# eldar/deepcut-cnn

Hardware: AMD Instinct MI355X
Metric: images/sec, DeeperCut ResNet-152 FCN forward (prob+loc_pred+next_pred), whole node (higher is better)
Workload: dtype f32

## Files before the change

deepcut-cnn_amd/csrc/c_api.cpp:

```cpp
#include <hip/hip_runtime_api.h>

#include <algorithm>
#include <cstdio>
#include <cstring>
#include <memory>
#include <string>
#include <vector>

#include "../../include/deepcut_hip.h"
#include "net.h"

using namespace dc;


namespace {
thread_local std::string g_err;
int fail(int code, const std::string& msg) {
  g_err = msg;
  return code;
}
template <typename F>
int guard(F&& f) {
  try {
    f();
// ... 581 lines not shown
const char* dc_conv_variant_name(int i) { return i >= 0 && i < dc::conv_num_variants() ? dc::conv_variant(i).name : nullptr; }
int dc_conv_variant_esize(int i) { return i >= 0 && i < dc::conv_num_variants() ? dc::conv_variant_esize(i) : 0; }
int dc_conv_bf16_variant_count(void) { return dc::conv_num_bf16_variants(); }
const char* dc_conv_bf16_variant_name(int i) {
  return i >= 0 && i < dc::conv_num_bf16_variants() ? dc::conv_variant(dc::kBf16Variant0 + i).name : nullptr;
}
int dc_wino_half_pack(const float* g, int cout, int cin, int rowscale, float* out, float* row_scale) {
  REQUIRE(g);
  REQUIRE(out);
  REQUIRE(row_scale);
  if (cout <= 0 || cin <= 0 || cout % 32 || cin % 16) return fail(DC_EINVAL, "dc_wino_half_pack: cout must be a multiple of 32, cin of 16");
  return guard([&] { dc::wino_half_pack_filters(g, cout, cin, rowscale != 0, out, row_scale); });
}

int dc_wino_blocks(const char* tile, int tiles_y, int tiles_x) {
  if (!tile || tiles_y < 1 || tiles_x < 1) return -1;
  try {
    return (int)dc::wino_form_blocks(dc::variant_by_name(tile), tiles_y, tiles_x);
  } catch (...) {
    return -1;
  }
}

int dc_stream1x1_pack(const float* g, int cout, int k, float* out) {
  if (!g || !out) return fail(DC_EINVAL, "dc_stream1x1_pack: null pointer");
  if (cout <= 0 || k <= 0 || cout % 32 || k % 16) return fail(DC_EINVAL, "dc_stream1x1_pack: cout must be a multiple of 32, k of 16");
  return guard([&] { dc::stream1x1_pack_filters(g, cout, k, out); });
}

int dc_stream1x1f_pack(const float* g, int cout, int k, float* out) {
  if (!g || !out) return fail(DC_EINVAL, "dc_stream1x1f_pack: null pointer");
  if (cout <= 0 || k <= 0 || cout % 16 || k % 16) return fail(DC_EINVAL, "dc_stream1x1f_pack: cout and k must be multiples of 16");
  return guard([&] { dc::stream1x1f_pack_filters(g, cout, k, out); });
}

int dc_stem7x7_pack(const float* g, int c, float* out) {
  if (!g || !out) return fail(DC_EINVAL, "dc_stem7x7_pack: null pointer");
  if (c < 1 || c > 4) return fail(DC_EINVAL, "dc_stem7x7_pack: 1 to 4 input channels");
  return guard([&] { dc::stem7x7_pack_filters(g, c, out); });
}

namespace {
inline NetGroup* G(dc_group* g) { return reinterpret_cast<NetGroup*>(g); }
}
int dc_group_create(dc_net* const* nets, int n, dc_group** out) {
  REQUIRE(nets);
// ... 206 lines not shown
```

deepcut-cnn_amd/csrc/forms.cpp:

```cpp
#include <cstring>
#include <string>

#include "kernels.h"

namespace dc {

static const char* const kWinoSlots[7] = {"index setup", "first loads issued", "two stages in LDS", "K loop", "partials to LDS + barrier",
                                          "inverse transform + epilogue constants", "shortcut + stores"};
static const char* const kStreamSlots[7] = {"prologue requests issued", "first stage + filters landed", "the first D steps", "the other steps",
                                            "drain", "-", "exit"};
static constexpr ConvForm kForms[kNumForms] = {
    {kWinoVariant, "wino_f23", "wino_f23<4x8x16>", kElemF32, kForm3x3, 8, kWinoSlots, wino_eligible, wino_grid, launch_wino_f23,
     false, false, nullptr, nullptr, kWinoVariant16, "DC_WINOGRAD"},
    {kWinoVariant16, "wino_f23_w16", "wino_f23<4x8x16_w16>", kElemF32, kForm3x3, 16, kWinoSlots, wino_eligible, wino_grid, launch_wino_f23_w16,
     false, false, nullptr, nullptr, kWinoVariant, "DC_WINOGRAD"},
    {kWinoHalf, "wino_h23", "wino_h23<2x4x8x64>", kElemF16, kForm3x3, 8, kWinoSlots, wino_half_eligible, wino_half_grid, launch_wino_half,
     true, true, nullptr, nullptr, -1, "DC_WINOGRAD"},
    {kStreamHalf, "ws1x1", "ws1x1<32xN>", kElemF16, kForm1x1, 4, kStreamSlots, stream1x1_eligible, stream1x1_grid, launch_stream1x1,
     false, true, stream1x1_prepare_multi, launch_stream1x1_multi, -1, "DC_STREAM1X1"},
    {kStemHalf, "stem7x7", "stem7x7<8x64>", kElemF16, kFormStem, 4, kWinoSlots, stem7x7_eligible, stem7x7_grid, launch_stem7x7,
     false, false, nullptr, nullptr, -1, "DC_STEM"},
    {kStreamFloat, "ws1x1f", "ws1x1f<16xN>", kElemF32, kForm1x1, 4, kStreamSlots, stream1x1f_eligible, stream1x1f_grid, launch_stream1x1f,
     false, true, nullptr, nullptr, -1, "DC_STREAM1X1"},
    {kStemFloat, "ws7x7f", "ws7x7f<16x64>", kElemF32, kFormStem, 4, kStreamSlots, stem_ws_eligible, stem_ws_grid, launch_stem_ws,
     false, true, nullptr, nullptr, -1, "DC_STEM"},
    {kWinoVariant56, "wino_f23_5x6", "wino_f23<5x6x16>", kElemF32, kForm3x3, 8, kWinoSlots, wino_eligible, wino_grid_5x6, launch_wino_f23_5x6,
     false, false, nullptr, nullptr, kWinoVariant56x16, "DC_WINOGRAD", wino_fewer_blocks},
    {kWinoVariant56x16, "wino_f23_5x6_w16", "wino_f23<5x6x16_w16>", kElemF32, kForm3x3, 16, kWinoSlots, wino_eligible, wino_grid_5x6, launch_wino_f23_5x6_w16,
     false, false, nullptr, nullptr, kWinoVariant56, "DC_WINOGRAD", wino_fewer_blocks},
    {kStreamBf16, "bs1x1", "bs1x1<32xN>", kElemBF16, kForm1x1, 4, kStreamSlots, stream1x1_bf16_eligible, stream1x1_grid, launch_stream1x1_bf16,
     false, true, stream1x1_bf16_prepare_multi, launch_stream1x1_bf16_multi, -1, "DC_STREAM1X1_BF16", nullptr, 0},
    {kStemBf16, "bs7x7", "bs7x7<8x64>", kElemBF16, kFormStem, 4, kWinoSlots, stem7x7_bf16_eligible, stem7x7_grid, launch_stem7x7_bf16,
     false, false, nullptr, nullptr, -1, "DC_STEM_BF16", nullptr, 0},
};

static constexpr bool forms_in_variant_order() {
  for (int i = 0; i < kNumForms; ++i)
    if (kForms[i].variant != kFormVariant0 + i) return false;
  return true;
}
static_assert(forms_in_variant_order(), "row i of kForms is variant kFormVariant0 + i");

const ConvForm* conv_form(int variant) {
  return variant >= kFormVariant0 && variant < kFormVariant0 + kNumForms ? &kForms[variant - kFormVariant0] : nullptr;
}

const char* variant_name(int v) {
  const ConvForm* f = conv_form(v);
  return f ? f->name : conv_variant(v).name;
}
int variant_by_name(const char* name) {
  for (const ConvForm& f : kForms)
    if (std::strcmp(name, f.name) == 0) return f.variant;
  return conv_variant_by_name(name);
}
std::string variant_kernel_label(int v) {
// ... 14 lines not shown
```

deepcut-cnn_amd/csrc/kernels.h:

```cpp
#pragma once
#include <cstddef>
#include <cstdint>
#include <string>

namespace dc {

constexpr int kMaxTaps = 32;

void dc_magic(unsigned d, unsigned (&mg)[2]);
bool xcd_map_on();

enum ElemKind { kElemF32 = 0, kElemF16 = 1, kElemBF16 = 2 };
inline int elem_kind_size(int kind) { return kind == kElemF32 ? 4 : 2; }
inline const char* elem_kind_name(int kind) { return kind == kElemF16 ? "f16" : kind == kElemBF16 ? "bf16" : "f32"; }

constexpr int kMaxClasses = 4;
struct ConvClass {
  int nty, ntx, dy0, ddy, x0, ddx, Ktot, x_bias;
  int OH, OW, M;
  int tiles_m;
  unsigned div_ohw[2];
  unsigned div_ow[2];
  long w_off;
  long y_off;
// ... 46 lines not shown
  int y_pix_stride;
  const void* resid;
  const float* scale;
  const float* shift;
  int relu;
  int sigmoid_ch;
  int xcd_on;
  int xcd_lgx;
  int tiles_m;
  unsigned div_rw[2][2];
  unsigned div_ohw[2];
  unsigned div_ow[2];
  unsigned div_tn[2];
  int tiles_n;
  long long* dbg;
  int w_TY, w_TX, w_NBY, w_NBX, w_nblk;
  unsigned w_div_nblk[2], w_div_nbyx[2], w_div_dd[2], w_div_d[2], w_div_nbx[2];
  int wide_epi;
  int vec_epi;
  int dense_x;
  int dense_y;
  int ncls;
  int mc_lgx;
  ConvClass cls[kMaxClasses];
  int nprob;
  int ekind;
};
struct ConvMultiArgs {
  ConvGemmParams p;
  ConvMultiTable t;
};
static_assert(sizeof(ConvMultiArgs) <= 4096, "HIP kernel arguments are limited to 4 KB");

struct ConvVariant {
  const char* name;
  int BM, BN, WR, WC, WK;
};
int conv_num_variants();
const ConvVariant& conv_variant(int i);
int conv_variant_bk(int i);
int conv_variant_esize(int i);
constexpr int kBf16Variant0 = 2000;
int conv_num_bf16_variants();
inline bool is_bf16_variant(int v) { return v >= kBf16Variant0 && v < kBf16Variant0 + conv_num_bf16_variants(); }
int conv_variant_ekind(int v);
bool conv_variant_exists(int v);
const int* conv_variants_of(int ekind, int* count);
int conv_variant_by_name(const char* name);
bool conv_variant_multiclass(int i);
long conv_grid(const ConvGemmParams& p, int variant);
int launch_conv_gemm(const ConvGemmParams& p, int variant, void* stream);
long prepare_conv_multi(ConvGemmParams& p, ConvMultiTable& table, int nprob, int variant);
bool conv_variant_multiproblem(int i);
int launch_conv_multi(const ConvMultiArgs& a, int variant, long grid, void* stream);

bool wino_eligible(const ConvGemmParams& p);
bool wino_same3x3(const ConvGemmParams& p);
ConvGemmParams wino_launch_params(const ConvGemmParams& p, long grid, int bty, int btx, int blocks_per_wg);
long wino_grid(const ConvGemmParams& p);
long wino_grid_5x6(const ConvGemmParams& p);
bool wino_fewer_blocks(const ConvGemmParams& p);
int launch_wino_f23(const ConvGemmParams& p, void* stream);
int launch_wino_f23_w16(const ConvGemmParams& p, void* stream);
int launch_wino_f23_5x6(const ConvGemmParams& p, void* stream);
int launch_wino_f23_5x6_w16(const ConvGemmParams& p, void* stream);
long wino_blocks(int TY, int TX, int bty, int btx);
long wino_form_blocks(int variant, int TY, int TX);
size_t wino_packed_floats(int Cout, int Cin);
void wino_pack_filters(const float* g, int Cout, int Cin, float* out);
bool wino_half_eligible(const ConvGemmParams& p);
long wino_half_grid(const ConvGemmParams& p);
size_t wino_half_packed_elems(int Cout, int Cin);
void wino_half_pack_filters(const float* g, int Cout, int Cin, bool rowscale, float* out, float* row_scale);
int launch_wino_half(const ConvGemmParams& p, void* stream);
bool stream1x1_eligible(const ConvGemmParams& p);
long stream1x1_grid(const ConvGemmParams& p);
size_t stream1x1_packed_elems(int Cout, int K);
void stream1x1_pack_filters(const float* g, int Cout, int K, float* out);
int launch_stream1x1(const ConvGemmParams& p, void* stream);
bool stream1x1f_eligible(const ConvGemmParams& p);
long stream1x1f_grid(const ConvGemmParams& p);
size_t stream1x1f_packed_elems(int Cout, int K);
void stream1x1f_pack_filters(const float* g, int Cout, int K, float* out);
int launch_stream1x1f(const ConvGemmParams& p, void* stream);
// ... 7 lines not shown
size_t stem7x7_packed_elems();
void stem7x7_pack_filters(const float* g, int C, float* out);
int launch_stem7x7(const ConvGemmParams& p, void* stream);
long stream1x1_prepare_multi(const ConvGemmParams& p, const ConvMultiTable& tb, int nprob);
int launch_stream1x1_multi(const ConvMultiArgs& a, void* stream);
bool stream1x1_bf16_eligible(const ConvGemmParams& p);
int launch_stream1x1_bf16(const ConvGemmParams& p, void* stream);
long stream1x1_bf16_prepare_multi(const ConvGemmParams& p, const ConvMultiTable& tb, int nprob);
int launch_stream1x1_bf16_multi(const ConvMultiArgs& a, void* stream);
bool stem7x7_bf16_eligible(const ConvGemmParams& p);
int launch_stem7x7_bf16(const ConvGemmParams& p, void* stream);

constexpr int kWinoVariant = 1000;
constexpr int kWinoVariant16 = 1001;
constexpr int kWinoHalf = 1002;
constexpr int kStreamHalf = 1003;
constexpr int kStemHalf = 1004;
constexpr int kStreamFloat = 1005;
constexpr int kStemFloat = 1006;
constexpr int kWinoVariant56 = 1007;
constexpr int kWinoVariant56x16 = 1008;
constexpr int kStreamBf16 = 1009;
constexpr int kStemBf16 = 1010;
constexpr int kFormVariant0 = kWinoVariant, kNumForms = 11;
enum FormGeometry { kForm3x3, kForm1x1, kFormStem };
struct ConvForm {
  int variant;
  const char *name, *label;
  int ekind, geometry, waves;
  const char* const* timing_slots;
  bool (*eligible)(const ConvGemmParams& p);
  long (*grid)(const ConvGemmParams& p);
  int (*launch)(const ConvGemmParams& p, void* stream);
  bool own_scale;
  bool merges;
  long (*prepare_multi)(const ConvGemmParams& p, const ConvMultiTable& tb, int nprob);
  int (*launch_multi)(const ConvMultiArgs& a, void* stream);
  int sibling;
  const char* env;
  bool (*offered)(const ConvGemmParams& p) = nullptr;
  int env_default = -1;
};
const ConvForm* conv_form(int variant);

const char* variant_name(int v);
int variant_by_name(const char* name);
std::string variant_kernel_label(int v);
// ... 97 lines not shown
```

deepcut-cnn_amd/csrc/wino_f32.hip:

```cpp
#include <hip/hip_runtime.h>

#include "conv_gemm.h"
#include "kernel_prims.h"
#include "kernels.h"

namespace dc {

namespace {
constexpr int WBTY = 4, WBTX = 8, WBN = 16, WKC = 32;
constexpr int WPSTR = WKC + 4;
constexpr int WPITCH = 672;
constexpr int WNTH = 512;
template <int FR_, int FC_, bool SIDE_, int PITCH_>
struct WinoGeom {
  static constexpr int FR = FR_, FC = FC_, NT = FR_ * FC_, PITCH = PITCH_;
  static constexpr bool SIDE = SIDE_;
  static constexpr int BTY = SIDE_ ? FR_ : 2 * FR_, BTX = SIDE_ ? 2 * FC_ : FC_;
  static constexpr int RH = 2 * BTY + 2, RW = 2 * BTX + 2;
  static constexpr int STAGE = RH * PITCH_ + 8;
  static constexpr int frow(int tf) { return SIDE_ ? 0 : FR_ * tf; }
  static constexpr int fcol(int tf) { return SIDE_ ? FC_ * tf : 0; }
  static constexpr int trow(int tf, int q) { return frow(tf) + q / FC_; }
  static constexpr int tcol(int tf, int q) { return fcol(tf) + q % FC_; }
  static constexpr bool conflict_free() {
    for (int tf = 0; tf < 2; ++tf)
      for (int flip = 0; flip < 2; ++flip) {
        bool seen[16] = {};
        for (int q = 0; q < NT; ++q) {
          const int slot = ((2 * trow(tf, q) * PITCH_ + 2 * tcol(tf, q) * WPSTR) / 4 + ((q >= 4 && q < 12) != (flip != 0) ? 1 : 0)) & 15;
          if (seen[slot]) return false;
          seen[slot] = true;
        }
      }
    return true;
  }
  static_assert(NT <= 16 && PITCH_ >= RW * WPSTR && WPSTR == 36 && conflict_free(), "conflict-free ds_read_b128 layout (see above)");
  static_assert(PITCH_ % 4 == 0 && WPSTR % 4 == 0 && STAGE % 4 == 0, "16-byte units");
};
using WinoG48 = WinoGeom<WBTY / 2, WBTX, false, WPITCH>;
using WinoG56 = WinoGeom<5, 3, true, 524>;
static_assert(WinoG48::BTY == 4 && WinoG48::BTX == 8 && WinoG48::RH == 10 && WinoG48::RW == 18, "the 4 x 8 block");
static_assert(WinoG56::BTY == 5 && WinoG56::BTX == 6 && WinoG56::RH == 12 && WinoG56::RW == 14, "the 5 x 6 block");
__device__ __forceinline__ f32x2 wlo(f32x4 v) { return __builtin_shufflevector(v, v, 0, 1); }
__device__ __forceinline__ f32x2 whi(f32x4 v) { return __builtin_shufflevector(v, v, 2, 3); }
}

template <int NG, class G>
__global__ __launch_bounds__(WNTH * NG, 4) void wino_f23_kernel(const ConvGemmParams p) {
  constexpr int NTH = WNTH * NG;
  constexpr int BTY = G::BTY, BTX = G::BTX, WRH = G::RH, WRW = G::RW, PITCH = G::PITCH, WSTAGE = G::STAGE;
  constexpr int WNLD = (WRH * WRW * (WKC / 4) + NTH - 1) / NTH;
  const long long t_entry = (long long)__builtin_amdgcn_s_memrealtime();
  DC_KARG_TOUCH(ka0, ka1, ka2, ka3, ka4);
  __shared__ __attribute__((aligned(16))) float stage[3][WSTAGE];
  float (*part)[4][2][2][4][64] = reinterpret_cast<float (*)[4][2][2][4][64]>(&stage[0][0]);
  static_assert(sizeof(float) * NG * 4 * 2 * 2 * 4 * 64 <= sizeof(stage), "partials must fit in the staging ring");
  static_assert(2 * sizeof(stage) <= 160 * 1024, "two workgroups per CU");
  const int t = threadIdx.x, lane = t & 63, wave = t >> 6;
  auto stamp = [&](int slot) {
    if (p.dbg && lane == 0) {
      long long* d = p.dbg + ((long)blockIdx.x * (8 * NG) + wave) * 12;
      d[slot] = (long long)__builtin_readcyclecounter();
      if (slot == 0) d[8] = t_entry, d[10] = (long long)__builtin_amdgcn_s_memrealtime();
      if (slot == 7) d[9] = (long long)__builtin_amdgcn_s_memrealtime();
    }
  };
  stamp(0);
  const int C = p.klen, H = p.x_rows, W = p.x_rowlen / p.klen;
  const int d = p.ddy;
  const int NBY = p.w_NBY, NBX = p.w_NBX;
  const int nblk = p.w_nblk;
  int lb = blockIdx.x;
  if (p.xcd_on) {
    const int g8 = gridDim.x >> 3, r8 = gridDim.x & 7, q = blockIdx.x & 7;
    lb = q * g8 + min(q, r8) + (blockIdx.x >> 3);
  }
  const int nt = dc_fastdiv(lb, p.w_div_nblk), blk = lb - nt * nblk;
  const int nph = dc_fastdiv(blk, p.w_div_nbyx), brem = blk - nph * (NBY * NBX);
  const int n = dc_fastdiv(nph, p.w_div_dd), ph = nph - n * (d * d);
  const int phy = dc_fastdiv(ph, p.w_div_d), phx = ph - phy * d;
  const int by = dc_fastdiv(brem, p.w_div_nbx), bx = brem - by * NBX;
  const int oy0 = 2 * BTY * by - 1, ox0 = 2 * BTX * bx - 1;
  DC_KARG_HOLD(ka0, ka1, ka2, ka3, ka4);
  const int kg = lane >> 4;
  const int grp = NG == 1 ? 0 : __builtin_amdgcn_readfirstlane(wave >> 3);
  const int i = wave & 3, tf = (wave >> 2) & 1;
  const int ra = i == 0 ? 0 : (i == 2 ? 2 : 1), rb = i == 0 ? 2 : (i == 1 ? 2 : (i == 2 ? 1 : 3));
  const float sb = i == 1 ? 1.f : -1.f;
  const __amdgpu_buffer_rsrc_t xr = dc_rsrc(reinterpret_cast<const float*>(p.x) + (long)n * p.x_img_stride, 0x7fffffffu);
  const __amdgpu_buffer_rsrc_t ur = dc_rsrc(p.w, 0x7fffffffu);
  unsigned gofs[WNLD];
  int sofs[WNLD];
#pragma unroll
  for (int q = 0; q < WNLD; ++q) {
    const int e = t + q * NTH;
    const int pix = e / (WKC / 4), cq = e % (WKC / 4);
    const int py = pix / WRW, px = pix % WRW;
    const int iy = phy + d * (oy0 + py), ix = phx + d * (ox0 + px);
    const bool ok = pix < WRH * WRW && oy0 + py >= 0 && ox0 + px >= 0 && iy < H && ix < W;
    gofs[q] = ok ? (unsigned)(iy * p.x_row_stride + ix * C + cq * 4) * 4u : kOOB;
    sofs[q] = (pix < WRH * WRW ? py * PITCH + px * WPSTR + cq * 4 : WSTAGE - 8 + (t & 1) * 4) >> 2;
  }
  const int qt = G::NT < 16 ? min(lane & 15, G::NT - 1) : lane & 15;
  const int r = qt / G::FC, c = G::fcol(tf) + qt % G::FC;
  const int ofs_a = (2 * (G::frow(tf) + r) + ra) * PITCH + 2 * c * WPSTR + kg * 4;
  const int ofs_b = (2 * (G::frow(tf) + r) + rb) * PITCH + 2 * c * WPSTR + kg * 4;
  f32x4 acc[4];
#pragma unroll
  for (int j = 0; j < 4; ++j) acc[j] = f32x4{0.f, 0.f, 0.f, 0.f};
  const unsigned uvo = ((unsigned)((nt * 4 + i) * (C / 16)) * (4 * 64 * 4) + (unsigned)lane * 4u) * 4u;
  f32x4 g[WNLD], b[2][4], da[4], db[4];
  auto gload = [&](int K) {
#pragma unroll
    for (int q = 0; q < WNLD; ++q) g[q] = dc_bload4(xr, gofs[q], (unsigned)(K * WKC * 4));
  };
  auto sstore = [&](int buf) {
#pragma unroll
    for (int q = 0; q < WNLD; ++q) reinterpret_cast<f32x4*>(&stage[buf][0])[sofs[q]] = g[q];
  };
  auto bload = [&](int slot, int k16) {
#pragma unroll
    for (int j = 0; j < 4; ++j) b[slot][j] = dc_bload4(ur, uvo + (unsigned)j * 1024u, (unsigned)k16 * 4096u);
  };
  auto lread = [&](int buf, int h) {
#pragma unroll
    for (int c4 = 0; c4 < 4; ++c4) {
      da[c4] = *reinterpret_cast<const f32x4*>(&stage[buf][ofs_a + c4 * WPSTR + h * 16]);
      db[c4] = *reinterpret_cast<const f32x4*>(&stage[buf][ofs_b + c4 * WPSTR + h * 16]);
    }
// ... 79 lines not shown
  stamp(4);
  __syncthreads();
#pragma unroll
  for (int r4 = 0; r4 < 4; ++r4) {
    part[grp][i][0][tf][r4][lane] = acc[0][r4] + acc[1][r4] + acc[2][r4];
    part[grp][i][1][tf][r4][lane] = acc[1][r4] - acc[2][r4] - acc[3][r4];
  }
  __syncthreads();
  stamp(5);
  const int a = (wave >> 1) & 1, bq = wave & 1;
  float* yb = reinterpret_cast<float*>(p.y);
  const float* rbp = reinterpret_cast<const float*>(p.resid);
  stamp(6);
#pragma unroll
  for (int rr = 0; rr < 4 / NG; ++rr) {
    const int r4 = NG == 1 ? rr : 2 * grp + rr;
    float p0 = part[0][0][bq][tf][r4][lane], p1 = part[0][1][bq][tf][r4][lane], p2 = part[0][2][bq][tf][r4][lane], p3 = part[0][3][bq][tf][r4][lane];
    if constexpr (NG == 2) {
      p0 += part[NG - 1][0][bq][tf][r4][lane], p1 += part[NG - 1][1][bq][tf][r4][lane];
      p2 += part[NG - 1][2][bq][tf][r4][lane], p3 += part[NG - 1][3][bq][tf][r4][lane];
    }
    float v = a == 0 ? p0 + p1 + p2 : p1 - p2 - p3;
    const int q = 4 * (lane >> 4) + r4;
    const int ty = by * BTY + G::frow(tf) + q / G::FC, tx = bx * BTX + G::fcol(tf) + q % G::FC;
    const int oy = phy + d * (2 * ty + a), ox = phx + d * (2 * tx + bq);
    if ((G::NT == 16 || q < G::NT) && oy < p.OH && ox < p.OW) {
      const long off = (long)n * p.y_img_stride + (long)oy * p.y_row_stride + (long)ox * p.y_pix_stride + co;
      v = v * sc + sh;
      if (rbp) v += rbp[off];
      if (p.relu) v = fmaxf(v, 0.f);
      yb[off] = v;
    }
  }
  stamp(7);
}

bool wino_same3x3(const ConvGemmParams& p) {
  const int d = p.ddy;
  if (p.nty != 3 || p.ntx != 3 || p.sy != 1 || d < 1 || d > 4 || p.dy0 != -d) return false;
  const int C = p.klen;
  if (C <= 0) return false;
  if (p.sx != C || p.ddx != d * C || p.x0 != -d * C) return false;
  if (p.x_rowlen % C != 0 || p.x_row_stride != p.x_rowlen) return false;
  return p.OH == p.x_rows && p.OW == p.x_rowlen / C;
}

ConvGemmParams wino_launch_params(const ConvGemmParams& p, long grid, int bty, int btx, int blocks_per_wg) {
  ConvGemmParams q = p;
  q.xcd_on = xcd_map_on() && grid >= 16;
// ... 9 lines not shown
  return q;
}

bool wino_eligible(const ConvGemmParams& p) {
  if (p.esize != 4 || !wino_same3x3(p)) return false;
  const int C = p.klen;
  if (C % WKC != 0 || p.Cout % WBN != 0 || p.sigmoid_ch != 0) return false;
  if ((long long)p.x_rows * p.x_row_stride * 4 >= 0x7fffffffLL || (long long)wino_packed_floats(p.Cout, C) * 4 >= 0x7fffffffLL) return false;
  return true;
}

long wino_blocks(int TY, int TX, int bty, int btx) { return (long)((TY + bty - 1) / bty) * ((TX + btx - 1) / btx); }

template <class G>
static long wino_grid_of(const ConvGemmParams& p) {
  const int d = p.ddy;
  const int TY = ((p.OH + d - 1) / d + 1) / 2, TX = ((p.OW + d - 1) / d + 1) / 2;
  return (long)p.NB * d * d * wino_blocks(TY, TX, G::BTY, G::BTX) * (p.Cout / WBN);
}
long wino_grid(const ConvGemmParams& p) { return wino_grid_of<WinoG48>(p); }
long wino_grid_5x6(const ConvGemmParams& p) { return wino_grid_of<WinoG56>(p); }

bool wino_fewer_blocks(const ConvGemmParams& p) { return wino_grid_of<WinoG56>(p) < wino_grid_of<WinoG48>(p); }

size_t wino_packed_floats(int Cout, int Cin) { return (size_t)16 * Cout * Cin; }

void wino_pack_filters(const float* g, int Cout, int Cin, float* out) {
  static const double G[4][3] = {{1, 0, 0}, {.5, .5, .5}, {.5, -.5, .5}, {0, 0, 1}};
  for (int co = 0; co < Cout; ++co)
    for (int ci = 0; ci < Cin; ++ci) {
      const float* w = g + ((size_t)co * Cin + ci) * 9;
      double tmp[4][3], U[4][4];
      for (int a = 0; a < 4; ++a)
        for (int b = 0; b < 3; ++b) tmp[a][b] = G[a][0] * w[b] + G[a][1] * w[3 + b] + G[a][2] * w[6 + b];
      for (int a = 0; a < 4; ++a)
        for (int b = 0; b < 4; ++b) U[a][b] = tmp[a][0] * G[b][0] + tmp[a][1] * G[b][1] + tmp[a][2] * G[b][2];
      const int nt = co / 16, col = co % 16, k16 = ci / 16, kg = (ci % 16) / 4, s = ci % 4;
      const int lane = kg * 16 + col;
      for (int i = 0; i < 4; ++i)
        for (int j = 0; j < 4; ++j)
          out[(((((size_t)nt * 4 + i) * (Cin / 16) + k16) * 4 + j) * 64 + lane) * 4 + s] = (float)U[i][j];
    }
}

template <int NG, class G>
static int launch_wino_f23(const ConvGemmParams& p, void* stream) {
  if (p.esize != 4 || !wino_eligible(p)) return (int)hipErrorInvalidValue;
  const long grid = wino_grid_of<G>(p);
  if (grid <= 0) return 0;
  if (grid > 0x7fffffffL) return (int)hipErrorInvalidValue;
  hipLaunchKernelGGL((wino_f23_kernel<NG, G>), dim3((unsigned)grid), dim3(NG * WNTH), 0, (hipStream_t)stream, wino_launch_params(p, grid, G::BTY, G::BTX, 1));
  return (int)hipGetLastError();
}
int launch_wino_f23(const ConvGemmParams& p, void* stream) { return launch_wino_f23<1, WinoG48>(p, stream); }
int launch_wino_f23_w16(const ConvGemmParams& p, void* stream) { return launch_wino_f23<2, WinoG48>(p, stream); }
int launch_wino_f23_5x6(const ConvGemmParams& p, void* stream) { return launch_wino_f23<1, WinoG56>(p, stream); }
int launch_wino_f23_5x6_w16(const ConvGemmParams& p, void* stream) { return launch_wino_f23<2, WinoG56>(p, stream); }

long wino_form_blocks(int variant, int TY, int TX) {
  if (variant == kWinoVariant || variant == kWinoVariant16) return wino_blocks(TY, TX, WinoG48::BTY, WinoG48::BTX);
  if (variant == kWinoVariant56 || variant == kWinoVariant56x16) return wino_blocks(TY, TX, WinoG56::BTY, WinoG56::BTX);
  return -1;
}

}
```

deepcut-cnn_amd/python/caffe/__init__.py:

```python
from .pycaffe import Net, NetGroup, Comm, Blob, Layer, choose_streams, pinned_empty, lpt_schedule, set_mode_cpu, set_mode_gpu, set_device, device_count, canvas_size, check_boxes, member_canvas, check_assembly, pair_stats_read, conv_variants, conv_variants_bf16, wino_half_pack, wino_blocks, stream1x1_pack, stream1x1f_pack, stem7x7_pack, lib_path
from .pycaffe import TRAIN, TEST, DeepcutError

__version__ = "1.0.0-rc3+deepcut_hip"
```

deepcut-cnn_amd/python/caffe/pycaffe.py:

```python
import ctypes as C
import os
import sys
from collections import OrderedDict

import numpy as np

TRAIN = 0
TEST = 1

_HERE = os.path.dirname(os.path.abspath(__file__))
_LIB_CANDIDATES = [
    os.environ.get("DEEPCUT_HIP_LIB", ""),
    os.path.normpath(os.path.join(_HERE, "..", "..", "lib", "libdeepcut_hip.so")),
]


class DeepcutError(RuntimeError):

    def __init__(self, code, msg):
        RuntimeError.__init__(self, msg)
        self.code = code


def lib_path():
# ... 117 lines not shown
        "dc_group_tune_report": (cp, [vp]),
        "dc_group_set_tile": (ci, [vp, cp, cp]),
        "dc_group_stats": (ci, [vp, C.POINTER(C.c_longlong), ci]),
        "dc_group_flops": (ci, [vp, C.POINTER(C.c_double)]),
        "dc_net_forward_host_async": (ci, [vp, vp, ci, ci, ci, vp, vp, vp]),
        "dc_host_alloc": (ci, [C.c_size_t, C.POINTER(vp)]),
        "dc_host_free": (ci, [vp]),
        "dc_nets_choose_streams": (ci, [C.POINTER(vp), ci, ci, ci, C.POINTER(C.c_double), C.POINTER(C.c_double)]),
        "dc_net_stream": (ci, [vp, C.POINTER(vp)]),
        "dc_comm_create": (ci, [ci, C.POINTER(ci), ci, C.POINTER(vp)]),
        "dc_comm_destroy": (ci, [vp]),
        "dc_comm_transport": (ci, [vp]),
        "dc_forward_batch": (ci, [vp, C.POINTER(vp), ci, C.POINTER(vp), C.POINTER(ci * 2), ci, C.POINTER(vp), C.POINTER(vp), C.POINTER(vp)]),
        "dc_comm_item_executor": (ci, [vp, ci]),
        "dc_comm_root_maps": (ci, [vp, ci, C.POINTER(vp), C.POINTER(vp), C.POINTER(vp), C.POINTER(ci)]),
        "dc_lpt_schedule": (ci, [C.POINTER(C.c_double), ci, ci, C.POINTER(ci)]),
        "dc_conv_variant_count": (ci, []),
        "dc_conv_variant_name": (cp, [ci]),
        "dc_conv_variant_esize": (ci, [ci]),
        "dc_conv_bf16_variant_count": (ci, []),
        "dc_conv_bf16_variant_name": (cp, [ci]),
        "dc_wino_half_pack": (ci, [C.c_void_p, ci, ci, ci, C.c_void_p, C.c_void_p]),
        "dc_wino_blocks": (ci, [cp, ci, ci]),
        "dc_stream1x1_pack": (ci, [C.c_void_p, ci, ci, C.c_void_p]),
        "dc_stem7x7_pack": (ci, [C.c_void_p, ci, C.c_void_p]),
        "dc_stream1x1f_pack": (ci, [C.c_void_p, ci, ci, C.c_void_p]),
    }
    for name, (res, args) in sig.items():
        fn = getattr(lib, name)
        fn.restype = res
        fn.argtypes = args
    return lib, sorted(sig)


_lib, EXPORTED_SYMBOLS = _load()


def _check(rc):
    if rc != 0:
        raise DeepcutError(rc, (_lib.dc_last_error() or b"").decode())


def set_mode_cpu():
    _check(_lib.dc_set_mode(0))


# ... 2 lines not shown


def set_device(device_id):
    _check(_lib.dc_set_device(int(device_id)))


def device_count():
    return _lib.dc_device_count()


_DTYPES = {"f32": 0, "float32": 0, "f16": 1, "float16": 1, "bf16": 2, "bfloat16": 2}


def conv_variants():
    return [((_lib.dc_conv_variant_name(i) or b"").decode(), _lib.dc_conv_variant_esize(i)) for i in range(_lib.dc_conv_variant_count())]


def conv_variants_bf16():
    return [(_lib.dc_conv_bf16_variant_name(i) or b"").decode() for i in range(_lib.dc_conv_bf16_variant_count())]


def wino_blocks(tile, tiles_y, tiles_x):
    return _lib.dc_wino_blocks(tile.encode(), int(tiles_y), int(tiles_x))


def stream1x1_pack(g):
    g = np.ascontiguousarray(g, np.float32)
    cout, k = g.shape[0], int(np.prod(g.shape[1:]))
    out = np.empty((cout // 32, k // 16, 64, 8), np.float32)
    _check(_lib.dc_stream1x1_pack(g.ctypes.data_as(C.c_void_p), cout, k, out.ctypes.data_as(C.c_void_p)))
    return out


def stream1x1f_pack(g):
    g = np.ascontiguousarray(g, np.float32)
    cout, k = g.shape[0], int(np.prod(g.shape[1:]))
    out = np.empty((cout // 16, k // 16, 64, 4), np.float32)
    _check(_lib.dc_stream1x1f_pack(g.ctypes.data_as(C.c_void_p), cout, k, out.ctypes.data_as(C.c_void_p)))
    return out


def stem7x7_pack(g):
    g = np.ascontiguousarray(g, np.float32)
    if g.ndim != 4 or g.shape[0] != 64 or g.shape[2:] != (7, 7):
        raise ValueError("stem7x7_pack: g must be [64, c, 7, 7]")
    out = np.empty((2, 7, 2, 64, 8), np.float32)
# ... 1042 lines not shown
```

deepcut-cnn_amd/python/deepcut_tools/tuning.py:

```python


_WINO_SIBLING = {"wino_f23": "wino_f23_w16", "wino_f23_w16": "wino_f23", "wino_f23_5x6": "wino_f23_5x6_w16", "wino_f23_5x6_w16": "wino_f23_5x6"}


def tune_in_flight(nets, run, top=6, margin=1.20, min_gain=0.01, reps=3, max_candidates=2, log=None):
    runs = [0]

    def measure():
        run()
        runs[0] += reps + 1
        return min(run() for _ in range(reps))

    before = incumbent = measure()
    report = nets[0].tune_report()
    have = [set(s["signature"] for s in n.tune_report()) for n in nets[1:]]
    ranked, skipped = [], 0
    for sig in report:
        if len(sig["timed"]) < 2 and sig["tile"] in _WINO_SIBLING:
            sig = dict(sig, timed=[(sig["tile"], 15.0), (_WINO_SIBLING[sig["tile"]], 15.0)])
        if len(sig["timed"]) < 2:
            skipped += 1
            continue
        if any(sig["signature"] not in h for h in have):
            skipped += 1
            continue
        alone = dict(sig["timed"])
        ranked.append((alone.get(sig["tile"], sig["timed"][0][1]) * sig["launches"], sig))
    ranked.sort(key=lambda t: -t[0])
    def put(signature, tile):
        for n in nets:
            n.set_tile(signature, tile)

    changed = []
    for _share, sig in ranked[:top]:
        best_alone = sig["timed"][0][1]
        cur = sig["tile"]
        keep = cur
        try:
            for tile, us in sig["timed"][:max_candidates + 1]:
                if tile == cur or us > margin * best_alone:
                    continue
                put(sig["signature"], tile)
                t = measure()
                if log:
                    log("  %-60s %-24s %.3f ms (incumbent %.3f)" % (sig["signature"][:60], tile, t * 1e3, incumbent * 1e3))
                if t < incumbent * (1.0 - min_gain):
                    put(sig["signature"], keep)
                    t_old = measure()
                    put(sig["signature"], tile)
                    t_new = measure()
                    if log:
                        log("    confirm: incumbent %.3f ms, candidate %.3f ms" % (t_old * 1e3, t_new * 1e3))
                    if t_new < t_old * (1.0 - min_gain):
                        changed.append((sig["signature"], keep, tile, t_old, t_new))
                        keep, incumbent = tile, t_new
                    else:
                        incumbent = min(incumbent, t_old)
        finally:
            put(sig["signature"], keep)
    after = measure() if changed else incumbent
    return {"before": before, "after": after, "changed": changed, "runs": runs[0], "skipped": skipped}
```

include/deepcut_hip.h:

```cpp
#ifndef DEEPCUT_HIP_H_
#define DEEPCUT_HIP_H_

#include <stddef.h>
#include <stdint.h>

#ifdef __cplusplus
extern "C" {
#endif

#define DC_OK 0
#define DC_EINVAL (-1)
#define DC_EIO (-2)
#define DC_ESHAPE (-3)
#define DC_EUNSUP (-4)
#define DC_EDEVICE (-5)
#define DC_ENOCPU (-6)

#define DC_MODE_CPU 0
#define DC_MODE_GPU 1
#define DC_PHASE_TRAIN 0
#define DC_PHASE_TEST 1

#define DC_OPT_FUSE 1
#define DC_OPT_HIPGRAPH 2
// ... 107 lines not shown
#define DC_STAT_LOWERINGS 0
#define DC_STAT_GRAPH_INSTANTIATIONS 1
#define DC_STAT_PLAN_HITS 2
#define DC_STAT_AUTOTUNE_RUNS 3
#define DC_STAT_BUFFER_GROWTHS 4
#define DC_STAT_REPACKS 5
#define DC_STAT_CACHED_PLANS 6
#define DC_NUM_STATS 7
int dc_net_stats(dc_net* net, long long* out, int n);
int dc_net_reserve(dc_net* net, int n, int h, int w);
int dc_net_device(dc_net* net);
const char* dc_net_plan_text(dc_net* net);
const char* dc_net_profile_text(dc_net* net, int iters);
const char* dc_net_debug_info(dc_net* net);
const char* dc_net_tune_report(dc_net* net);
int dc_net_set_tile(dc_net* net, const char* signature, const char* tile);
int dc_conv_variant_count(void);
const char* dc_conv_variant_name(int i);
int dc_conv_variant_esize(int i);
int dc_conv_bf16_variant_count(void);
const char* dc_conv_bf16_variant_name(int i);
int dc_wino_half_pack(const float* g, int cout, int cin, int rowscale, float* out, float* row_scale);
int dc_wino_blocks(const char* tile, int tiles_y, int tiles_x);

int dc_stream1x1_pack(const float* g, int cout, int k, float* out);
int dc_stem7x7_pack(const float* g, int c, float* out);
int dc_stream1x1f_pack(const float* g, int cout, int k, float* out);

typedef struct dc_group dc_group;
int dc_group_create(dc_net* const* nets, int n, dc_group** out);
int dc_group_destroy(dc_group* group);
int dc_group_size(dc_group* group);
int dc_group_set_lanes(dc_group* group, int lanes);
int dc_group_forward_batch(dc_group* group, const float* const* inputs, const int* n, const int* h, const int* w, int is_device,
                           float* const* prob, float* const* loc_pred, float* const* next_pred, void* stream);
int dc_group_forward_images(dc_group* group, const unsigned char* const* images, const int* n, const int* height, const int* width,
                            const double* scale, int is_device, float* const* prob, float* const* loc_pred, float* const* next_pred,
                            double* const* pose, void* stream);
int dc_group_forward_boxes(dc_group* group, const unsigned char* image, int height, int width, int is_device, const int* boxes,
                           const double* scales, int n, const double* pyramid_scales, int canvas_h, int canvas_w, float* const* prob,
                           float* const* loc_pred, float* const* next_pred, double* const* pose, void* stream);
int dc_group_fuse_maps(dc_group* group, const double* scales, int base, int n_edges, const double* mean, const double* stdev, float* prob,
                       float* loc_pred, float* next_pred, int is_device, void* stream);
int dc_group_detect_parts(dc_group* group, const double* scales, int base, float threshold, int radius, int max_det, int* counts,
                          double* dets);
int dc_group_assemble_people(dc_group* group, const double* scales, int base, const dc_assemble_params* p, int n_edges, const int* edges,
// ... 52 lines not shown
```

Baseline: 532.3.

## Add mixed 4x8 + 5x6 Winograd block cover to cut padded tiles

Adds a Winograd F(2,3) kernel variant that splits the output tile grid at a horizontal or vertical cut. One part is covered with 4x8 blocks and the rest with 5x6 blocks, and the split is chosen to minimise the total block count. This targets work wasted on partially filled edge blocks when neither block shape divides the grid well. The cost is extra per-block branching, index setup for two geometries, and one more kernel-argument line. The in-flight tuner is also widened so it times Winograd sibling variants beyond the top candidates, which is how the new form would get selected.

After: 543.4, median of 6. 1.02x the previous value.

```diff
diff --git a/deepcut-cnn_amd/csrc/c_api.cpp b/deepcut-cnn_amd/csrc/c_api.cpp
--- a/deepcut-cnn_amd/csrc/c_api.cpp
+++ b/deepcut-cnn_amd/csrc/c_api.cpp
@@ -627,6 +627,19 @@
   }
 }
 
+int dc_wino_cover(int tiles_y, int tiles_x, int* out) {
+  if (!out || tiles_y < 1 || tiles_x < 1) return -1;
+  const dc::WinoCover c = dc::wino_plan_cover(tiles_y, tiles_x);
+  const int v[12] = {c.vertical, c.cut, c.blocks, c.na, c.nb, c.a_nby, c.a_nbx, c.b_nby, c.b_nbx, c.b_ty0, c.b_tx0, dc::wino_mix_offered(tiles_y, tiles_x) ? 1 : 0};
+  for (int i = 0; i < 12; ++i) out[i] = v[i];
+  return c.blocks;
+}
+
+int dc_wino_mix_offered(int tiles_y, int tiles_x, int images, int cout) {
+  if (tiles_y < 1 || tiles_x < 1 || images < 1 || cout < 1) return -1;
+  return dc::wino_mix_offered_launch(tiles_y, tiles_x, images, cout) ? 1 : 0;
+}
+
 int dc_stream1x1_pack(const float* g, int cout, int k, float* out) {
   if (!g || !out) return fail(DC_EINVAL, "dc_stream1x1_pack: null pointer");
   if (cout <= 0 || k <= 0 || cout % 32 || k % 16) return fail(DC_EINVAL, "dc_stream1x1_pack: cout must be a multiple of 32, k of 16");
diff --git a/deepcut-cnn_amd/csrc/forms.cpp b/deepcut-cnn_amd/csrc/forms.cpp
--- a/deepcut-cnn_amd/csrc/forms.cpp
+++ b/deepcut-cnn_amd/csrc/forms.cpp
@@ -32,6 +32,10 @@
      false, true, stream1x1_bf16_prepare_multi, launch_stream1x1_bf16_multi, -1, "DC_STREAM1X1_BF16", nullptr, 0},
     {kStemBf16, "bs7x7", "bs7x7<8x64>", kElemBF16, kFormStem, 4, kWinoSlots, stem7x7_bf16_eligible, stem7x7_grid, launch_stem7x7_bf16,
      false, false, nullptr, nullptr, -1, "DC_STEM_BF16", nullptr, 0},
+    {kWinoVariantMix, "wino_f23_mix", "wino_f23<4x8+5x6x16>", kElemF32, kForm3x3, 8, kWinoSlots, wino_eligible, wino_grid_mix, launch_wino_f23_mix,
+     false, false, nullptr, nullptr, kWinoVariantMix16, "DC_WINOGRAD", wino_mix_fewer_blocks},
+    {kWinoVariantMix16, "wino_f23_mix_w16", "wino_f23<4x8+5x6x16_w16>", kElemF32, kForm3x3, 16, kWinoSlots, wino_eligible, wino_grid_mix, launch_wino_f23_mix_w16,
+     false, false, nullptr, nullptr, kWinoVariantMix, "DC_WINOGRAD", wino_mix_fewer_blocks},
 };
 
 static constexpr bool forms_in_variant_order() {
diff --git a/deepcut-cnn_amd/csrc/kernels.h b/deepcut-cnn_amd/csrc/kernels.h
--- a/deepcut-cnn_amd/csrc/kernels.h
+++ b/deepcut-cnn_amd/csrc/kernels.h
@@ -92,10 +92,17 @@
   int dense_y;
   int ncls;
   int mc_lgx;
+  int w_mix_pad_;
+  int w_mix_na, w_mix_nab, w_mix_ty0, w_mix_tx0, w_mix_NBX;
+  unsigned w_mix_div_nbx[2];
+  int w_mix_reserved_[8];
   ConvClass cls[kMaxClasses];
   int nprob;
   int ekind;
 };
+static_assert(offsetof(ConvGemmParams, w_mix_na) % 64 == 0 && offsetof(ConvGemmParams, w_mix_div_nbx) + 8 <= offsetof(ConvGemmParams, w_mix_na) + 64 &&
+                  offsetof(ConvGemmParams, cls) == offsetof(ConvGemmParams, w_mix_na) + 64,
+              "the w_mix_* fields are one 64-byte line of the argument block, the multi-class table starts on the next");
 struct ConvMultiArgs {
   ConvGemmParams p;
   ConvMultiTable t;
@@ -130,6 +137,16 @@
 long wino_grid(const ConvGemmParams& p);
 long wino_grid_5x6(const ConvGemmParams& p);
 bool wino_fewer_blocks(const ConvGemmParams& p);
+struct WinoCover {
+  int vertical, cut, blocks, na, nb, a_nby, a_nbx, b_nby, b_nbx, b_ty0, b_tx0;
+};
+WinoCover wino_plan_cover(int TY, int TX);
+long wino_grid_mix(const ConvGemmParams& p);
+bool wino_mix_offered(int TY, int TX);
+bool wino_mix_offered_launch(int TY, int TX, long images, int Cout);
+bool wino_mix_fewer_blocks(const ConvGemmParams& p);
+int launch_wino_f23_mix(const ConvGemmParams& p, void* stream);
+int launch_wino_f23_mix_w16(const ConvGemmParams& p, void* stream);
 int launch_wino_f23(const ConvGemmParams& p, void* stream);
 int launch_wino_f23_w16(const ConvGemmParams& p, void* stream);
 int launch_wino_f23_5x6(const ConvGemmParams& p, void* stream);
@@ -183,7 +200,9 @@
 constexpr int kWinoVariant56x16 = 1008;
 constexpr int kStreamBf16 = 1009;
 constexpr int kStemBf16 = 1010;
-constexpr int kFormVariant0 = kWinoVariant, kNumForms = 11;
+constexpr int kWinoVariantMix = 1011;
+constexpr int kWinoVariantMix16 = 1012;
+constexpr int kFormVariant0 = kWinoVariant, kNumForms = 13;
 enum FormGeometry { kForm3x3, kForm1x1, kFormStem };
 struct ConvForm {
   int variant;
diff --git a/deepcut-cnn_amd/csrc/wino_f32.hip b/deepcut-cnn_amd/csrc/wino_f32.hip
--- a/deepcut-cnn_amd/csrc/wino_f32.hip
+++ b/deepcut-cnn_amd/csrc/wino_f32.hip
@@ -1,4 +1,6 @@
 #include <hip/hip_runtime.h>
+
+#include <algorithm>
 
 #include "conv_gemm.h"
 #include "kernel_prims.h"
@@ -18,6 +20,8 @@
   static constexpr int BTY = SIDE_ ? FR_ : 2 * FR_, BTX = SIDE_ ? 2 * FC_ : FC_;
   static constexpr int RH = 2 * BTY + 2, RW = 2 * BTX + 2;
   static constexpr int STAGE = RH * PITCH_ + 8;
+  static constexpr int PIXELS = RH * RW;
+  static constexpr bool MIX = false;
   static constexpr int frow(int tf) { return SIDE_ ? 0 : FR_ * tf; }
   static constexpr int fcol(int tf) { return SIDE_ ? FC_ * tf : 0; }
   static constexpr int trow(int tf, int q) { return frow(tf) + q / FC_; }
@@ -41,6 +45,10 @@
 using WinoG56 = WinoGeom<5, 3, true, 524>;
 static_assert(WinoG48::BTY == 4 && WinoG48::BTX == 8 && WinoG48::RH == 10 && WinoG48::RW == 18, "the 4 x 8 block");
 static_assert(WinoG56::BTY == 5 && WinoG56::BTX == 6 && WinoG56::RH == 12 && WinoG56::RW == 14, "the 5 x 6 block");
+struct WinoGMix {
+  static constexpr int STAGE = std::max(WinoG48::STAGE, WinoG56::STAGE), PIXELS = std::max(WinoG48::PIXELS, WinoG56::PIXELS);
+  static constexpr bool MIX = true;
+};
 __device__ __forceinline__ f32x2 wlo(f32x4 v) { return __builtin_shufflevector(v, v, 0, 1); }
 __device__ __forceinline__ f32x2 whi(f32x4 v) { return __builtin_shufflevector(v, v, 2, 3); }
 }
@@ -48,10 +56,12 @@
 template <int NG, class G>
 __global__ __launch_bounds__(WNTH * NG, 4) void wino_f23_kernel(const ConvGemmParams p) {
   constexpr int NTH = WNTH * NG;
-  constexpr int BTY = G::BTY, BTX = G::BTX, WRH = G::RH, WRW = G::RW, PITCH = G::PITCH, WSTAGE = G::STAGE;
-  constexpr int WNLD = (WRH * WRW * (WKC / 4) + NTH - 1) / NTH;
+  constexpr int WSTAGE = G::STAGE;
+  constexpr int WNLD = (G::PIXELS * (WKC / 4) + NTH - 1) / NTH;
   const long long t_entry = (long long)__builtin_amdgcn_s_memrealtime();
   DC_KARG_TOUCH(ka0, ka1, ka2, ka3, ka4);
+  unsigned ka5 = 0;
+  if constexpr (G::MIX) asm volatile("s_load_dword %0, %1, %2" : "=&s"(ka5) : "s"(__builtin_amdgcn_kernarg_segment_ptr()), "n"(offsetof(ConvGemmParams, w_mix_na)));
   __shared__ __attribute__((aligned(16))) float stage[3][WSTAGE];
   float (*part)[4][2][2][4][64] = reinterpret_cast<float (*)[4][2][2][4][64]>(&stage[0][0]);
   static_assert(sizeof(float) * NG * 4 * 2 * 2 * 4 * 64 <= sizeof(stage), "partials must fit in the staging ring");
@@ -76,12 +86,23 @@
     lb = q * g8 + min(q, r8) + (blockIdx.x >> 3);
   }
   const int nt = dc_fastdiv(lb, p.w_div_nblk), blk = lb - nt * nblk;
-  const int nph = dc_fastdiv(blk, p.w_div_nbyx), brem = blk - nph * (NBY * NBX);
+  const int nph = dc_fastdiv(blk, p.w_div_nbyx), brem = blk - nph * (G::MIX ? p.w_mix_nab : NBY * NBX);
   const int n = dc_fastdiv(nph, p.w_div_dd), ph = nph - n * (d * d);
   const int phy = dc_fastdiv(ph, p.w_div_d), phx = ph - phy * d;
-  const int by = dc_fastdiv(brem, p.w_div_nbx), bx = brem - by * NBX;
-  const int oy0 = 2 * BTY * by - 1, ox0 = 2 * BTX * bx - 1;
+  bool in_b = false;
+  int by, bx, rty0 = 0, rtx0 = 0, oy0, ox0;
+  if constexpr (G::MIX) {
+    in_b = brem >= p.w_mix_na;
+    const int br = in_b ? brem - p.w_mix_na : brem;
+    by = in_b ? dc_fastdiv(br, p.w_mix_div_nbx) : dc_fastdiv(br, p.w_div_nbx), bx = br - by * (in_b ? p.w_mix_NBX : NBX);
+    rty0 = in_b ? p.w_mix_ty0 : 0, rtx0 = in_b ? p.w_mix_tx0 : 0;
+    oy0 = 2 * (rty0 + (in_b ? WinoG56::BTY : WinoG48::BTY) * by) - 1, ox0 = 2 * (rtx0 + (in_b ? WinoG56::BTX : WinoG48::BTX) * bx) - 1;
+  } else {
+    by = dc_fastdiv(brem, p.w_div_nbx), bx = brem - by * NBX;
+    oy0 = 2 * G::BTY * by - 1, ox0 = 2 * G::BTX * bx - 1;
+  }
   DC_KARG_HOLD(ka0, ka1, ka2, ka3, ka4);
+  if constexpr (G::MIX) asm volatile("" ::"s"(ka5));
   const int kg = lane >> 4;
   const int grp = NG == 1 ? 0 : __builtin_amdgcn_readfirstlane(wave >> 3);
   const int i = wave & 3, tf = (wave >> 2) & 1;
@@ -90,21 +111,46 @@
   const __amdgpu_buffer_rsrc_t xr = dc_rsrc(reinterpret_cast<const float*>(p.x) + (long)n * p.x_img_stride, 0x7fffffffu);
   const __amdgpu_buffer_rsrc_t ur = dc_rsrc(p.w, 0x7fffffffu);
   unsigned gofs[WNLD];
-  int sofs[WNLD];
-#pragma unroll
-  for (int q = 0; q < WNLD; ++q) {
-    const int e = t + q * NTH;
-    const int pix = e / (WKC / 4), cq = e % (WKC / 4);
-    const int py = pix / WRW, px = pix % WRW;
-    const int iy = phy + d * (oy0 + py), ix = phx + d * (ox0 + px);
-    const bool ok = pix < WRH * WRW && oy0 + py >= 0 && ox0 + px >= 0 && iy < H && ix < W;
-    gofs[q] = ok ? (unsigned)(iy * p.x_row_stride + ix * C + cq * 4) * 4u : kOOB;
-    sofs[q] = (pix < WRH * WRW ? py * PITCH + px * WPSTR + cq * 4 : WSTAGE - 8 + (t & 1) * 4) >> 2;
-  }
-  const int qt = G::NT < 16 ? min(lane & 15, G::NT - 1) : lane & 15;
-  const int r = qt / G::FC, c = G::fcol(tf) + qt % G::FC;
-  const int ofs_a = (2 * (G::frow(tf) + r) + ra) * PITCH + 2 * c * WPSTR + kg * 4;
-  const int ofs_b = (2 * (G::frow(tf) + r) + rb) * PITCH + 2 * c * WPSTR + kg * 4;
+  int sofs[WNLD], ofs_a, ofs_b;
+  if constexpr (!G::MIX) {
+#pragma unroll
+    for (int q = 0; q < WNLD; ++q) {
+      const int e = t + q * NTH;
+      const int pix = e / (WKC / 4), cq = e % (WKC / 4);
+      const int py = pix / G::RW, px = pix % G::RW;
+      const int iy = phy + d * (oy0 + py), ix = phx + d * (ox0 + px);
+      const bool ok = pix < G::PIXELS && oy0 + py >= 0 && ox0 + px >= 0 && iy < H && ix < W;
+      gofs[q] = ok ? (unsigned)(iy * p.x_row_stride + ix * C + cq * 4) * 4u : kOOB;
+      sofs[q] = (pix < G::PIXELS ? py * G::PITCH + px * WPSTR + cq * 4 : WSTAGE - 8 + (t & 1) * 4) >> 2;
+    }
+    const int qt = G::NT < 16 ? min(lane & 15, G::NT - 1) : lane & 15;
+    const int r = qt / G::FC, c = G::fcol(tf) + qt % G::FC;
+    ofs_a = (2 * (G::frow(tf) + r) + ra) * G::PITCH + 2 * c * WPSTR + kg * 4;
+    ofs_b = (2 * (G::frow(tf) + r) + rb) * G::PITCH + 2 * c * WPSTR + kg * 4;
+  } else {
+    auto index_setup = [&](auto geom) {
+      using GG = decltype(geom);
+  #pragma unroll
+      for (int q = 0; q < WNLD; ++q) {
+        const int e = t + q * NTH;
+        const int pix = e / (WKC / 4), cq = e % (WKC / 4);
+        const int py = pix / GG::RW, px = pix % GG::RW;
+        const int iy = phy + d * (oy0 + py), ix = phx + d * (ox0 + px);
+        const bool ok = pix < GG::PIXELS && oy0 + py >= 0 && ox0 + px >= 0 && iy < H && ix < W;
+        gofs[q] = ok ? (unsigned)(iy * p.x_row_stride + ix * C + cq * 4) * 4u : kOOB;
+        sofs[q] = (pix < GG::PIXELS ? py * GG::PITCH + px * WPSTR + cq * 4 : GG::STAGE - 8 + (t & 1) * 4) >> 2;
+      }
+      const int qt = GG::NT < 16 ? min(lane & 15, GG::NT - 1) : lane & 15;
+      const int r = qt / GG::FC, c = GG::fcol(tf) + qt % GG::FC;
+      ofs_a = (2 * (GG::frow(tf) + r) + ra) * GG::PITCH + 2 * c * WPSTR + kg * 4;
+      ofs_b = (2 * (GG::frow(tf) + r) + rb) * GG::PITCH + 2 * c * WPSTR + kg * 4;
+    };
+    if (in_b)
+      index_setup(WinoG56{});
+    else
+      index_setup(WinoG48{});
+    __builtin_assume((ofs_a & 3) == 0 && (ofs_b & 3) == 0);
+  }
   f32x4 acc[4];
 #pragma unroll
   for (int j = 0; j < 4; ++j) acc[j] = f32x4{0.f, 0.f, 0.f, 0.f};
@@ -230,9 +276,23 @@
     }
     float v = a == 0 ? p0 + p1 + p2 : p1 - p2 - p3;
     const int q = 4 * (lane >> 4) + r4;
-    const int ty = by * BTY + G::frow(tf) + q / G::FC, tx = bx * BTX + G::fcol(tf) + q % G::FC;
+    int ty, tx;
+    bool has_tile;
+    auto tile_of = [&](auto geom) {
+      using GG = decltype(geom);
+      ty = rty0 + by * GG::BTY + GG::frow(tf) + q / GG::FC, tx = rtx0 + bx * GG::BTX + GG::fcol(tf) + q % GG::FC;
+      has_tile = GG::NT == 16 || q < GG::NT;
+    };
+    if constexpr (G::MIX) {
+      if (in_b)
+        tile_of(WinoG56{});
+      else
+        tile_of(WinoG48{});
+    } else {
+      tile_of(G{});
+    }
     const int oy = phy + d * (2 * ty + a), ox = phx + d * (2 * tx + bq);
-    if ((G::NT == 16 || q < G::NT) && oy < p.OH && ox < p.OW) {
+    if (has_tile && oy < p.OH && ox < p.OW) {
       const long off = (long)n * p.y_img_stride + (long)oy * p.y_row_stride + (long)ox * p.y_pix_stride + co;
       v = v * sc + sh;
       if (rbp) v += rbp[off];
@@ -288,6 +348,46 @@
 long wino_grid_5x6(const ConvGemmParams& p) { return wino_grid_of<WinoG56>(p); }
 
 bool wino_fewer_blocks(const ConvGemmParams& p) { return wino_grid_of<WinoG56>(p) < wino_grid_of<WinoG48>(p); }
+
+WinoCover wino_plan_cover(int TY, int TX) {
+  WinoCover best{};
+  best.blocks = -1;
+  for (int vertical = 0; vertical < 2; ++vertical) {
+    const int ext = vertical ? TX : TY, step = vertical ? WinoG48::BTX : WinoG48::BTY;
+    for (int cut = 0; cut <= ext; cut = cut == ext ? ext + 1 : std::min(cut + step, ext)) {
+      WinoCover c{};
+      c.vertical = vertical, c.cut = cut;
+      const int aty = vertical ? TY : cut, atx = vertical ? cut : TX, bty = vertical ? TY : TY - cut, btx = vertical ? TX - cut : TX;
+      if (aty > 0 && atx > 0) c.a_nby = (aty + WinoG48::BTY - 1) / WinoG48::BTY, c.a_nbx = (atx + WinoG48::BTX - 1) / WinoG48::BTX;
+      if (bty > 0 && btx > 0) c.b_nby = (bty + WinoG56::BTY - 1) / WinoG56::BTY, c.b_nbx = (btx + WinoG56::BTX - 1) / WinoG56::BTX;
+      c.na = c.a_nby * c.a_nbx, c.nb = c.b_nby * c.b_nbx, c.blocks = c.na + c.nb;
+      c.b_ty0 = vertical ? 0 : cut, c.b_tx0 = vertical ? cut : 0;
+      const bool is_cut = c.na > 0 && c.nb > 0, best_cut = best.na > 0 && best.nb > 0;
+      if (best.blocks < 0 || c.blocks < best.blocks || (c.blocks == best.blocks && (is_cut < best_cut || (is_cut == best_cut && c.nb < best.nb)))) best = c;
+    }
+  }
+  return best;
+}
+static long wino_mix_grid_tiles(const ConvGemmParams& p, int& TY, int& TX) {
+  const int d = p.ddy;
+  TY = ((p.OH + d - 1) / d + 1) / 2, TX = ((p.OW + d - 1) / d + 1) / 2;
+  return (long)p.NB * d * d * wino_plan_cover(TY, TX).blocks * (p.Cout / WBN);
+}
+long wino_grid_mix(const ConvGemmParams& p) {
+  int TY, TX;
+  return wino_mix_grid_tiles(p, TY, TX);
+}
+bool wino_mix_offered(int TY, int TX) {
+  return wino_plan_cover(TY, TX).blocks < std::min(wino_blocks(TY, TX, WinoG48::BTY, WinoG48::BTX), wino_blocks(TY, TX, WinoG56::BTY, WinoG56::BTX));
+}
+constexpr long kWinoMixMinWorkgroups = 128;
+bool wino_mix_offered_launch(int TY, int TX, long images, int Cout) {
+  return wino_mix_offered(TY, TX) && images * wino_blocks(TY, TX, WinoG48::BTY, WinoG48::BTX) * (Cout / WBN) >= kWinoMixMinWorkgroups;
+}
+bool wino_mix_fewer_blocks(const ConvGemmParams& p) {
+  int TY, TX;
+  return wino_mix_grid_tiles(p, TY, TX) > 0 && wino_mix_offered_launch(TY, TX, (long)p.NB * p.ddy * p.ddy, p.Cout);
+}
 
 size_t wino_packed_floats(int Cout, int Cin) { return (size_t)16 * Cout * Cin; }
 
@@ -323,9 +423,32 @@
 int launch_wino_f23_5x6(const ConvGemmParams& p, void* stream) { return launch_wino_f23<1, WinoG56>(p, stream); }
 int launch_wino_f23_5x6_w16(const ConvGemmParams& p, void* stream) { return launch_wino_f23<2, WinoG56>(p, stream); }
 
+template <int NG>
+static int launch_wino_f23_mix(const ConvGemmParams& p, void* stream) {
+  if (p.esize != 4 || !wino_eligible(p)) return (int)hipErrorInvalidValue;
+  int TY, TX;
+  const long grid = wino_mix_grid_tiles(p, TY, TX);
+  if (grid <= 0) return 0;
+  if (grid > 0x7fffffffL) return (int)hipErrorInvalidValue;
+  const WinoCover c = wino_plan_cover(TY, TX);
+  ConvGemmParams q = wino_launch_params(p, grid, WinoG48::BTY, WinoG48::BTX, 1);
+  q.w_NBY = c.a_nby, q.w_NBX = c.a_nbx;
+  q.w_nblk = p.NB * p.ddy * p.ddy * c.blocks;
+  q.w_mix_na = c.na, q.w_mix_nab = c.blocks, q.w_mix_ty0 = c.b_ty0, q.w_mix_tx0 = c.b_tx0, q.w_mix_NBX = c.b_nbx;
+  dc_magic((unsigned)q.w_nblk, q.w_div_nblk);
+  dc_magic((unsigned)c.blocks, q.w_div_nbyx);
+  dc_magic((unsigned)c.a_nbx, q.w_div_nbx);
+  dc_magic((unsigned)c.b_nbx, q.w_mix_div_nbx);
+  hipLaunchKernelGGL((wino_f23_kernel<NG, WinoGMix>), dim3((unsigned)grid), dim3(NG * WNTH), 0, (hipStream_t)stream, q);
+  return (int)hipGetLastError();
+}
+int launch_wino_f23_mix(const ConvGemmParams& p, void* stream) { return launch_wino_f23_mix<1>(p, stream); }
+int launch_wino_f23_mix_w16(const ConvGemmParams& p, void* stream) { return launch_wino_f23_mix<2>(p, stream); }
+
 long wino_form_blocks(int variant, int TY, int TX) {
   if (variant == kWinoVariant || variant == kWinoVariant16) return wino_blocks(TY, TX, WinoG48::BTY, WinoG48::BTX);
   if (variant == kWinoVariant56 || variant == kWinoVariant56x16) return wino_blocks(TY, TX, WinoG56::BTY, WinoG56::BTX);
+  if (variant == kWinoVariantMix || variant == kWinoVariantMix16) return wino_plan_cover(TY, TX).blocks;
   return -1;
 }
 
diff --git a/deepcut-cnn_amd/python/caffe/__init__.py b/deepcut-cnn_amd/python/caffe/__init__.py
--- a/deepcut-cnn_amd/python/caffe/__init__.py
+++ b/deepcut-cnn_amd/python/caffe/__init__.py
@@ -1,4 +1,4 @@
-from .pycaffe import Net, NetGroup, Comm, Blob, Layer, choose_streams, pinned_empty, lpt_schedule, set_mode_cpu, set_mode_gpu, set_device, device_count, canvas_size, check_boxes, member_canvas, check_assembly, pair_stats_read, conv_variants, conv_variants_bf16, wino_half_pack, wino_blocks, stream1x1_pack, stream1x1f_pack, stem7x7_pack, lib_path
+from .pycaffe import Net, NetGroup, Comm, Blob, Layer, choose_streams, pinned_empty, lpt_schedule, set_mode_cpu, set_mode_gpu, set_device, device_count, canvas_size, check_boxes, member_canvas, check_assembly, pair_stats_read, conv_variants, conv_variants_bf16, wino_half_pack, wino_blocks, wino_cover, wino_mix_offered, stream1x1_pack, stream1x1f_pack, stem7x7_pack, lib_path
 from .pycaffe import TRAIN, TEST, DeepcutError
 
 __version__ = "1.0.0-rc3+deepcut_hip"
diff --git a/deepcut-cnn_amd/python/caffe/pycaffe.py b/deepcut-cnn_amd/python/caffe/pycaffe.py
--- a/deepcut-cnn_amd/python/caffe/pycaffe.py
+++ b/deepcut-cnn_amd/python/caffe/pycaffe.py
@@ -163,6 +163,8 @@
         "dc_conv_bf16_variant_name": (cp, [ci]),
         "dc_wino_half_pack": (ci, [C.c_void_p, ci, ci, ci, C.c_void_p, C.c_void_p]),
         "dc_wino_blocks": (ci, [cp, ci, ci]),
+        "dc_wino_cover": (ci, [ci, ci, C.c_void_p]),
+        "dc_wino_mix_offered": (ci, [ci, ci, ci, ci]),
         "dc_stream1x1_pack": (ci, [C.c_void_p, ci, ci, C.c_void_p]),
         "dc_stem7x7_pack": (ci, [C.c_void_p, ci, C.c_void_p]),
         "dc_stream1x1f_pack": (ci, [C.c_void_p, ci, ci, C.c_void_p]),
@@ -211,6 +213,18 @@
 
 def wino_blocks(tile, tiles_y, tiles_x):
     return _lib.dc_wino_blocks(tile.encode(), int(tiles_y), int(tiles_x))
+
+
+def wino_cover(tiles_y, tiles_x):
+    out = (C.c_int * 12)()
+    if _lib.dc_wino_cover(int(tiles_y), int(tiles_x), C.cast(out, C.c_void_p)) < 0:
+        return None
+    keys = ("vertical", "cut", "blocks", "na", "nb", "a_nby", "a_nbx", "b_nby", "b_nbx", "b_ty0", "b_tx0", "offered")
+    return dict(zip(keys, (int(v) for v in out)))
+
+
+def wino_mix_offered(tiles_y, tiles_x, images, cout):
+    return _lib.dc_wino_mix_offered(int(tiles_y), int(tiles_x), int(images), int(cout))
 
 
 def stream1x1_pack(g):
diff --git a/deepcut-cnn_amd/python/deepcut_tools/tuning.py b/deepcut-cnn_amd/python/deepcut_tools/tuning.py
--- a/deepcut-cnn_amd/python/deepcut_tools/tuning.py
+++ b/deepcut-cnn_amd/python/deepcut_tools/tuning.py
@@ -1,6 +1,7 @@
 
 
-_WINO_SIBLING = {"wino_f23": "wino_f23_w16", "wino_f23_w16": "wino_f23", "wino_f23_5x6": "wino_f23_5x6_w16", "wino_f23_5x6_w16": "wino_f23_5x6"}
+_WINO_SIBLING = {"wino_f23": "wino_f23_w16", "wino_f23_w16": "wino_f23", "wino_f23_5x6": "wino_f23_5x6_w16", "wino_f23_5x6_w16": "wino_f23_5x6",
+                 "wino_f23_mix": "wino_f23_mix_w16", "wino_f23_mix_w16": "wino_f23_mix"}
 
 
 def tune_in_flight(nets, run, top=6, margin=1.20, min_gain=0.01, reps=3, max_candidates=2, log=None):
@@ -37,7 +38,8 @@
         cur = sig["tile"]
         keep = cur
         try:
-            for tile, us in sig["timed"][:max_candidates + 1]:
+            family = [c for c in sig["timed"][max_candidates + 1:] if c[0] in _WINO_SIBLING]
+            for tile, us in sig["timed"][:max_candidates + 1] + family:
                 if tile == cur or us > margin * best_alone:
                     continue
                 put(sig["signature"], tile)
diff --git a/include/deepcut_hip.h b/include/deepcut_hip.h
--- a/include/deepcut_hip.h
+++ b/include/deepcut_hip.h
@@ -153,6 +153,8 @@
 const char* dc_conv_bf16_variant_name(int i);
 int dc_wino_half_pack(const float* g, int cout, int cin, int rowscale, float* out, float* row_scale);
 int dc_wino_blocks(const char* tile, int tiles_y, int tiles_x);
+int dc_wino_cover(int tiles_y, int tiles_x, int* out);
+int dc_wino_mix_offered(int tiles_y, int tiles_x, int images, int cout);
 
 int dc_stream1x1_pack(const float* g, int cout, int k, float* out);
 int dc_stem7x7_pack(const float* g, int c, float* out);
```
